# Kmatsuo57/cell-image-analysis

Measured on AMD Instinct MI355X. Metric: cells/sec screened (CAE fwd + recon-MSE + SVM score), 64x64, higher is better.
Workload: dtype f32 (results in the fp32 error class; the contractions run as split 16-bit products on the matrix pipe, fp32 accumulate: conv1..conv6 as 2 fp16 terms x 3 products with exact power-of-two scales from each cell's own data, the PCA GEMM as 3 bf16 terms x 6 products, conv7's 32 -> 16 channel contraction; 1 GPU; BASELINE.json configs[2]: screening inference, 1000000 synthetic 64x64 crops on one GPU, resident in HBM, CAE fwd + recon MSE/MAE + RobustScaler + PCA(100) + 2x OCSVM score on device; cells_per_gpu=1000000, global_cells=1000000, chunk_cells=65536, detector_train_cells=5000, weights=random init (Glorot, non-trivial BN), seed 42, parallelism=dp1

## Files before the change

cell-image-analysis_amd/csrc/conv45_h2.hip:

```cpp
#include "common.hpp"

#include <cstring>

namespace cs {

namespace {

constexpr int G = 8;
constexpr int CH = 32;
constexpr int WP = G + 2;
constexpr int PXB = 64;
constexpr int ROWB = WP * PXB + 32;
constexpr int PLANE = WP * ROWB;
constexpr int WG_PER_CU = 2;

constexpr int C5_OUT = 64;

typedef _Float16 f16x8 __attribute__((ext_vector_type(8)));
typedef _Float16 f16x4 __attribute__((ext_vector_type(4)));
constexpr int H2_OFF_MAX = 2 * PLANE;
constexpr int H2_LDS_BYTES = 2 * PLANE + 16;

__device__ __forceinline__ unsigned int h2_rowmax(unsigned int m)
{
    unsigned int o;
    o = (unsigned int)__builtin_amdgcn_update_dpp(0, (int)m, 0xB1, 0xF, 0xF, true);  m = m > o ? m : o;
    o = (unsigned int)__builtin_amdgcn_update_dpp(0, (int)m, 0x4E, 0xF, 0xF, true);  m = m > o ? m : o;
    o = (unsigned int)__builtin_amdgcn_update_dpp(0, (int)m, 0x124, 0xF, 0xF, true); m = m > o ? m : o;
    o = (unsigned int)__builtin_amdgcn_update_dpp(0, (int)m, 0x128, 0xF, 0xF, true); m = m > o ? m : o;
    return m;
}
__device__ __forceinline__ void h2_scale(unsigned int mbits, float& S, float& invS)
{
    int E = (int)((mbits >> 23) & 0xffu);
    E = E < 40 ? 40 : (E > 254 ? 254 : E);
    S = __builtin_bit_cast(float, (unsigned int)(268 - E) << 23);
    invS = __builtin_bit_cast(float, (unsigned int)(E - 14) << 23);
}
__device__ __forceinline__ void h2_absmax4(const f32x4& v, unsigned int& mx)
{
    const float a = v[0], b = v[1], c = v[2], d = v[3];
    const float m = fmaxf(fmaxf(fabsf(a), fabsf(b)), fmaxf(fabsf(c), fabsf(d)));
    const unsigned int u = __builtin_bit_cast(unsigned int, m);
    mx = mx > u ? mx : u;
}
__device__ __forceinline__ void h2_split_store(char* dst, const f32x4& x, float S)
{
    const f32x4 v = x * S;
    const f16x4 hi = __builtin_convertvector(v, f16x4);
    const f32x4 r = v - __builtin_convertvector(hi, f32x4);
    *(f16x4*)dst = hi;
    *(f16x4*)(dst + PLANE) = __builtin_convertvector(r, f16x4);
}

__global__ __launch_bounds__(256, WG_PER_CU) void conv4_h2_kernel(const float* __restrict__ in, const f16x8* __restrict__ wfrag,
                                                                 const float* __restrict__ ep, float* __restrict__ out,
                                                                 long n_cells, float inv_sw)
{
    extern __shared__ __attribute__((aligned(16))) char smem[];
    unsigned int* const mxw = (unsigned int*)(smem + H2_OFF_MAX);
    const int tid = threadIdx.x;
    const int lane = tid & 63;
    const int wave = __builtin_amdgcn_readfirstlane(tid >> 6);
    const int slice = wave & 1;
    const int th = wave >> 1;
    const int li = lane & 15, kq = lane >> 4;

    f16x8 B[9][2];
#pragma unroll
    for (int t = 0; t < 9; ++t)
#pragma unroll
        for (int p = 0; p < 2; ++p) B[t][p] = wfrag[((slice * 9 + t) * 2 + p) * 64 + lane];
    const int co = slice * 16 + li;
    const float bias = ep[co], bns = ep[CH + co], bnt = ep[2 * CH + co];

    for (int i = tid; i < H2_LDS_BYTES / 16; i += 256) *(f32x4*)(smem + i * 16) = f32x4{0.0f, 0.0f, 0.0f, 0.0f};

    long cell = blockIdx.x;
    if (cell >= n_cells) return;
    f32x4 stg[2];
#pragma unroll
    for (int k = 0; k < 2; ++k) stg[k] = *(const f32x4*)(in + (size_t)cell * (G * G * CH) + (tid + 256 * k) * 4);
    __syncthreads();
    {
        unsigned int mx = 0;
        h2_absmax4(stg[0], mx);
        h2_absmax4(stg[1], mx);
        mx = h2_rowmax(mx);
        if (li == 0) atomicMax(&mxw[0], mx);
    }
    __syncthreads();
    float S, invS;
    h2_scale(mxw[0], S, invS);

    int woff[2];
#pragma unroll
    for (int k = 0; k < 2; ++k) {
        const int idx = tid + 256 * k, px = idx >> 3, c4 = idx & 7;
        woff[k] = ((px >> 3) + 1) * ROWB + ((px & 7) + 1) * PXB + c4 * 8;
    }
    const int abase = (4 * th + (li >> 3)) * ROWB + (li & 7) * PXB + kq * 16;

    for (int it = 0; cell < n_cells; cell += gridDim.x, ++it) {
        const float unscale = invS * inv_sw;
#pragma unroll
        for (int k = 0; k < 2; ++k) h2_split_store(smem + woff[k], stg[k], S);
        __syncthreads();
        if (tid == 0) mxw[it & 1] = 0;
        const long ncell = cell + gridDim.x;
        if (ncell < n_cells) {
#pragma unroll
            for (int k = 0; k < 2; ++k) stg[k] = *(const f32x4*)(in + (size_t)ncell * (G * G * CH) + (tid + 256 * k) * 4);
        }

        f32x4 hi[2] = {{0.0f, 0.0f, 0.0f, 0.0f}, {0.0f, 0.0f, 0.0f, 0.0f}};
        f32x4 lo[2] = {{0.0f, 0.0f, 0.0f, 0.0f}, {0.0f, 0.0f, 0.0f, 0.0f}};
#pragma unroll
        for (int tap = 0; tap < 9; ++tap) {
            const int toff = (tap / 3) * ROWB + (tap % 3) * PXB;
#pragma unroll
            for (int t = 0; t < 2; ++t) {
                const char* a = smem + abase + toff + t * (2 * ROWB);
                const f16x8 a1 = *(const f16x8*)a;
                const f16x8 a2 = *(const f16x8*)(a + PLANE);
                lo[t] = __builtin_amdgcn_mfma_f32_16x16x32_f16(a1, B[tap][1], lo[t], 0, 0, 0);
                hi[t] = __builtin_amdgcn_mfma_f32_16x16x32_f16(a1, B[tap][0], hi[t], 0, 0, 0);
                lo[t] = __builtin_amdgcn_mfma_f32_16x16x32_f16(a2, B[tap][0], lo[t], 0, 0, 0);
            }
        }
#pragma unroll
        for (int t = 0; t < 2; ++t) {
            float* o = out + ((size_t)cell * (G * G) + 16 * (2 * th + t) + 4 * kq) * CH + co;
#pragma unroll
            for (int r = 0; r < 4; ++r) {
                const float v = fmaxf(fmaf(hi[t][r] + lo[t][r], unscale, bias), 0.0f);
                o[r * CH] = fmaf(v, bns, bnt);
            }
        }
        if (ncell < n_cells) {
            unsigned int mx = 0;
            h2_absmax4(stg[0], mx);
            h2_absmax4(stg[1], mx);
            mx = h2_rowmax(mx);
            if (li == 0) atomicMax(&mxw[(it + 1) & 1], mx);
        }
        __syncthreads();
        h2_scale(mxw[(it + 1) & 1], S, invS);
    }
}

__global__ __launch_bounds__(512, 2) void conv5_h2_kernel(const float* __restrict__ in, const f16x8* __restrict__ wfrag,
                                                          const float* __restrict__ ep, float* __restrict__ out, long n_cells, float inv_sw)
{
    extern __shared__ __attribute__((aligned(16))) char smem[];
    unsigned int* const mxw = (unsigned int*)(smem + H2_OFF_MAX);
    const int tid = threadIdx.x;
    const int lane = tid & 63;
    const int wave = __builtin_amdgcn_readfirstlane(tid >> 6);
    const int ph = wave >> 1, pa = ph >> 1, pb = ph & 1;
    const int sp = wave & 1;
    const int li = lane & 15, kq = lane >> 4;

    f16x8 B[4][2][2];
#pragma unroll
    for (int t = 0; t < 4; ++t)
#pragma unroll
        for (int k = 0; k < 2; ++k)
#pragma unroll
            for (int p = 0; p < 2; ++p) B[t][k][p] = wfrag[(((wave * 4 + t) * 2 + k) * 2 + p) * 64 + lane];
    float bias[2], bns[2], bnt[2];
#pragma unroll
    for (int k = 0; k < 2; ++k) {
        const int co = (2 * sp + k) * 16 + li;
        bias[k] = ep[co]; bns[k] = ep[C5_OUT + co]; bnt[k] = ep[2 * C5_OUT + co];
    }

    for (int i = tid; i < H2_LDS_BYTES / 16; i += 512) *(f32x4*)(smem + i * 16) = f32x4{0.0f, 0.0f, 0.0f, 0.0f};

    long cell = blockIdx.x;
    if (cell >= n_cells) return;
    f32x4 stg = *(const f32x4*)(in + (size_t)cell * (G * G * CH) + tid * 4);
    __syncthreads();
    {
        unsigned int mx = 0;
        h2_absmax4(stg, mx);
        mx = h2_rowmax(mx);
        if (li == 0) atomicMax(&mxw[0], mx);
    }
    __syncthreads();
    float S, invS;
    h2_scale(mxw[0], S, invS);
    const int woff = ((tid >> 6) + 1) * ROWB + (((tid >> 3) & 7) + 1) * PXB + (tid & 7) * 8;
    const int abase = ((li >> 3) + pa) * ROWB + ((li & 7) + pb) * PXB + kq * 16;

    for (int it = 0; cell < n_cells; cell += gridDim.x, ++it) {
        const float unscale = invS * inv_sw;
        h2_split_store(smem + woff, stg, S);
        __syncthreads();
        if (tid == 0) mxw[it & 1] = 0;
        const long ncell = cell + gridDim.x;
        if (ncell < n_cells) stg = *(const f32x4*)(in + (size_t)ncell * (G * G * CH) + tid * 4);

        float* obase = out + (((size_t)cell * (2 * G) + pa) * (2 * G) + pb) * C5_OUT + (2 * sp) * 16 + li;
#pragma unroll
        for (int t = 0; t < 4; ++t) {
            f32x4 ah[2] = {{0.0f, 0.0f, 0.0f, 0.0f}, {0.0f, 0.0f, 0.0f, 0.0f}};
            f32x4 al[2] = {{0.0f, 0.0f, 0.0f, 0.0f}, {0.0f, 0.0f, 0.0f, 0.0f}};
#pragma unroll
            for (int tap = 0; tap < 4; ++tap) {
                const char* a = smem + abase + t * (2 * ROWB) + (tap >> 1) * ROWB + (tap & 1) * PXB;
                const f16x8 a1 = *(const f16x8*)a;
                const f16x8 a2 = *(const f16x8*)(a + PLANE);
#pragma unroll
                for (int k = 0; k < 2; ++k) {
                    al[k] = __builtin_amdgcn_mfma_f32_16x16x32_f16(a1, B[tap][k][1], al[k], 0, 0, 0);
                    ah[k] = __builtin_amdgcn_mfma_f32_16x16x32_f16(a1, B[tap][k][0], ah[k], 0, 0, 0);
                    al[k] = __builtin_amdgcn_mfma_f32_16x16x32_f16(a2, B[tap][k][0], al[k], 0, 0, 0);
                }
            }
#pragma unroll
            for (int r = 0; r < 4; ++r) {
                const int i = 4 * kq + r, ys = 2 * t + (i >> 3), xs = i & 7;
                float* o = obase + ((size_t)(2 * ys) * (2 * G) + 2 * xs) * C5_OUT;
#pragma unroll
                for (int k = 0; k < 2; ++k) {
                    const float v = fmaxf(fmaf(ah[k][r] + al[k][r], unscale, bias[k]), 0.0f);
                    o[16 * k] = fmaf(v, bns[k], bnt[k]);
                }
            }
        }
        if (ncell < n_cells) {
            unsigned int mx = 0;
            h2_absmax4(stg, mx);
            mx = h2_rowmax(mx);
            if (li == 0) atomicMax(&mxw[(it + 1) & 1], mx);
        }
        __syncthreads();
        h2_scale(mxw[(it + 1) & 1], S, invS);
    }
}

constexpr int F45_OFF_A = 2 * PLANE;
constexpr int F45_OFF_W4 = 4 * PLANE;
constexpr int F45_W4_BYTES = 2 * 9 * 2 * 64 * 16;
constexpr int F45_OFF_MAX = F45_OFF_W4 + F45_W4_BYTES;
constexpr int F45_LDS_BYTES = F45_OFF_MAX + 16;
static_assert(2 * F45_LDS_BYTES <= 160 * 1024, "two workgroups per CU");

__global__ __launch_bounds__(512, 2) void conv45_h2_kernel(const float* __restrict__ in , const f16x8* __restrict__ w4frag,
                                                           const float* __restrict__ ep4, float inv_sw4, const f16x8* __restrict__ w5frag,
                                                           const float* __restrict__ ep5, float inv_sw5, float* __restrict__ out ,
                                                           long n_cells)
{
    extern __shared__ __attribute__((aligned(16))) char smem[];
    unsigned int* const mxw = (unsigned int*)(smem + F45_OFF_MAX);
    const int tid = threadIdx.x;
    const int lane = tid & 63;
    const int wave = __builtin_amdgcn_readfirstlane(tid >> 6);
    const int li = lane & 15, kq = lane >> 4;
    const int ph = wave >> 1, pa = ph >> 1, pb = ph & 1;
    const int sp = wave & 1;
    const int slice4 = wave & 1, tile4 = wave >> 1;

    f16x8 B[4][2][2];
#pragma unroll
    for (int t = 0; t < 4; ++t)
#pragma unroll
        for (int k = 0; k < 2; ++k)
#pragma unroll
            for (int p = 0; p < 2; ++p) B[t][k][p] = w5frag[(((wave * 4 + t) * 2 + k) * 2 + p) * 64 + lane];
    float bias[2], bns[2], bnt[2];
#pragma unroll
    for (int k = 0; k < 2; ++k) {
        const int co = (2 * sp + k) * 16 + li;
        bias[k] = ep5[co]; bns[k] = ep5[C5_OUT + co]; bnt[k] = ep5[2 * C5_OUT + co];
    }
    const int co4 = slice4 * 16 + li;
    const float bias4 = ep4[co4], bns4 = ep4[CH + co4], bnt4 = ep4[2 * CH + co4];

    for (int i = tid; i < F45_LDS_BYTES / 16; i += 512) *(f32x4*)(smem + i * 16) = f32x4{0.0f, 0.0f, 0.0f, 0.0f};
    __syncthreads();
    for (int i = tid; i < F45_W4_BYTES / 16; i += 512) *(f16x8*)(smem + F45_OFF_W4 + i * 16) = w4frag[i];

    long cell = blockIdx.x;
    if (cell >= n_cells) return;
    f32x4 stg = *(const f32x4*)(in + (size_t)cell * (G * G * CH) + tid * 4);
    {
        unsigned int mx = 0;
        h2_absmax4(stg, mx);
        mx = h2_rowmax(mx);
        if (li == 0) atomicMax(&mxw[0], mx);
    }
    __syncthreads();
    float S3, invS3;
    h2_scale(mxw[0], S3, invS3);
    const int woff = ((tid >> 6) + 1) * ROWB + (((tid >> 3) & 7) + 1) * PXB + (tid & 7) * 8;
    const int abase4 = (2 * tile4 + (li >> 3)) * ROWB + (li & 7) * PXB + kq * 16;
    const char* const w4l = smem + F45_OFF_W4 + (size_t)slice4 * 9 * 2 * 64 * 16 + lane * 16;
    const int abase5 = F45_OFF_A + ((li >> 3) + pa) * ROWB + ((li & 7) + pb) * PXB + kq * 16;

    for (int it = 0; cell < n_cells; cell += gridDim.x, ++it) {
        h2_split_store(smem + woff, stg, S3);
        __syncthreads();
        if (tid == 0) mxw[it & 1] = 0;
        const long ncell = cell + gridDim.x;
        if (ncell < n_cells) stg = *(const f32x4*)(in + (size_t)ncell * (G * G * CH) + tid * 4);

        f32x4 a4v;
        {
            f32x4 hi = {0.0f, 0.0f, 0.0f, 0.0f}, lo = {0.0f, 0.0f, 0.0f, 0.0f};
#pragma unroll
            for (int tap = 0; tap < 9; ++tap) {
                const char* a = smem + abase4 + (tap / 3) * ROWB + (tap % 3) * PXB;
                const f16x8 a1 = *(const f16x8*)a;
                const f16x8 a2 = *(const f16x8*)(a + PLANE);
                const f16x8 bh = *(const f16x8*)(w4l + (tap * 2 + 0) * 1024), bl = *(const f16x8*)(w4l + (tap * 2 + 1) * 1024);
                lo = __builtin_amdgcn_mfma_f32_16x16x32_f16(a1, bl, lo, 0, 0, 0);
                hi = __builtin_amdgcn_mfma_f32_16x16x32_f16(a1, bh, hi, 0, 0, 0);
                lo = __builtin_amdgcn_mfma_f32_16x16x32_f16(a2, bh, lo, 0, 0, 0);
            }
            const float us4 = invS3 * inv_sw4;
            float am = 0.0f;
#pragma unroll
            for (int r = 0; r < 4; ++r) {
                const float v = fmaxf(fmaf(hi[r] + lo[r], us4, bias4), 0.0f);
                a4v[r] = fmaf(v, bns4, bnt4);
                am = fmaxf(am, fabsf(a4v[r]));
            }
            const unsigned int m = h2_rowmax(__builtin_bit_cast(unsigned int, am));
            if (li == 0) atomicMax(&mxw[2 + (it & 1)], m);
        }
        __syncthreads();
        float S4, invS4;
        h2_scale(mxw[2 + (it & 1)], S4, invS4);
        {
#pragma unroll
            for (int r = 0; r < 4; ++r) {
                const int p = 16 * tile4 + 4 * kq + r;
                char* d = smem + F45_OFF_A + ((p >> 3) + 1) * ROWB + ((p & 7) + 1) * PXB + co4 * 2;
                const float v = a4v[r] * S4;
                const _Float16 h = (_Float16)v;
                *(_Float16*)d = h;
                *(_Float16*)(d + PLANE) = (_Float16)(v - (float)h);
            }
        }
        __syncthreads();
        if (tid == 0) mxw[2 + (it & 1)] = 0;

        const float unscale = invS4 * inv_sw5;
        float* obase = out + (((size_t)cell * (2 * G) + pa) * (2 * G) + pb) * C5_OUT + (2 * sp) * 16 + li;
#pragma unroll
        for (int t = 0; t < 4; ++t) {
            f32x4 ah[2] = {{0.0f, 0.0f, 0.0f, 0.0f}, {0.0f, 0.0f, 0.0f, 0.0f}};
            f32x4 al[2] = {{0.0f, 0.0f, 0.0f, 0.0f}, {0.0f, 0.0f, 0.0f, 0.0f}};
#pragma unroll
            for (int tap = 0; tap < 4; ++tap) {
                const char* a = smem + abase5 + t * (2 * ROWB) + (tap >> 1) * ROWB + (tap & 1) * PXB;
                const f16x8 a1 = *(const f16x8*)a;
                const f16x8 a2 = *(const f16x8*)(a + PLANE);
#pragma unroll
                for (int k = 0; k < 2; ++k) {
                    al[k] = __builtin_amdgcn_mfma_f32_16x16x32_f16(a1, B[tap][k][1], al[k], 0, 0, 0);
                    ah[k] = __builtin_amdgcn_mfma_f32_16x16x32_f16(a1, B[tap][k][0], ah[k], 0, 0, 0);
                    al[k] = __builtin_amdgcn_mfma_f32_16x16x32_f16(a2, B[tap][k][0], al[k], 0, 0, 0);
                }
            }
#pragma unroll
            for (int r = 0; r < 4; ++r) {
                const int i = 4 * kq + r, ys = 2 * t + (i >> 3), xs = i & 7;
                float* o = obase + ((size_t)(2 * ys) * (2 * G) + 2 * xs) * C5_OUT;
#pragma unroll
                for (int k = 0; k < 2; ++k) {
                    const float v = fmaxf(fmaf(ah[k][r] + al[k][r], unscale, bias[k]), 0.0f);
                    o[16 * k] = fmaf(v, bns[k], bnt[k]);
                }
            }
        }
        if (ncell < n_cells) {
            unsigned int mx = 0;
            h2_absmax4(stg, mx);
            mx = h2_rowmax(mx);
            if (li == 0) atomicMax(&mxw[(it + 1) & 1], mx);
        }
        __syncthreads();
        h2_scale(mxw[(it + 1) & 1], S3, invS3);
    }
}

}

size_t pack_conv4_f16x2(const float* hwio, uint16_t* dst, float* inv_sw)
{
    const size_t n = (size_t)2 * 9 * 2 * 64 * 8;
    if (!dst) return n;
    const float S = f16x2_weight_scale(hwio, (size_t)9 * CH * CH);
    if (inv_sw) *inv_sw = 1.0f / S;
    for (int s = 0; s < 2; ++s)
        for (int t = 0; t < 9; ++t)
            for (int l = 0; l < 64; ++l)
                for (int j = 0; j < 8; ++j) {
                    const int li = l & 15, kq = l >> 4;
                    uint16_t pl[2];
                    f16x2_split(hwio[((size_t)t * CH + 8 * kq + j) * CH + 16 * s + li], S, pl[0], pl[1]);
                    for (int p = 0; p < 2; ++p) dst[((((size_t)s * 9 + t) * 2 + p) * 64 + l) * 8 + j] = pl[p];
                }
    return n;
}

template <class K>
static hipError_t resident_grid(K kernel, int threads, int lds, int& resident)
{
    int dev = 0, cus = 0, per_cu = 0;
    hipError_t e;
    if ((e = hipGetDevice(&dev)) != hipSuccess) return e;
    if ((e = hipDeviceGetAttribute(&cus, hipDeviceAttributeMultiprocessorCount, dev)) != hipSuccess) return e;
    if ((e = hipOccupancyMaxActiveBlocksPerMultiprocessor(&per_cu, (const void*)kernel, threads, lds)) != hipSuccess) return e;
    resident = cus * (per_cu < 1 ? 1 : per_cu);
    return hipSuccess;
}

hipError_t launch_conv4_h2(const float* in, const uint16_t* wfrag, float inv_sw, const float* ep, float* out, int64_t n_cells, hipStream_t stream)
{
    if (n_cells <= 0) return hipSuccess;
    static int resident = 0;
    if (!resident) {
        hipError_t e = resident_grid(conv4_h2_kernel, 256, H2_LDS_BYTES, resident);
        if (e != hipSuccess) return e;
    }
    const long grid = n_cells < resident ? n_cells : resident;
    hipLaunchKernelGGL(conv4_h2_kernel, dim3((unsigned)grid), dim3(256), H2_LDS_BYTES, stream, in, (const f16x8*)wfrag, ep, out,
                       (long)n_cells, inv_sw);
    return hipGetLastError();
}

size_t pack_conv5_f16x2(const float* weff, uint16_t* dst, float* inv_sw)
{
    const size_t n = (size_t)8 * 4 * 2 * 2 * 64 * 8;
    if (!dst) return n;
    const float S = f16x2_weight_scale(weff, (size_t)16 * CH * C5_OUT);
    if (inv_sw) *inv_sw = 1.0f / S;
    for (int w = 0; w < 8; ++w)
        for (int t = 0; t < 4; ++t)
            for (int k = 0; k < 2; ++k)
                for (int l = 0; l < 64; ++l)
                    for (int j = 0; j < 8; ++j) {
                        const int ph = w >> 1, sp = w & 1, li = l & 15, kq = l >> 4;
                        uint16_t pl[2];
                        f16x2_split(weff[((size_t)(ph * 4 + t) * CH + 8 * kq + j) * C5_OUT + (2 * sp + k) * 16 + li], S, pl[0], pl[1]);
                        for (int p = 0; p < 2; ++p) dst[((((((size_t)w * 4 + t) * 2 + k) * 2 + p) * 64) + l) * 8 + j] = pl[p];
                    }
    return n;
}

hipError_t launch_conv5_h2(const float* in, const uint16_t* wfrag, float inv_sw, const float* ep, float* out, int64_t n_cells, hipStream_t stream)
{
    if (n_cells <= 0) return hipSuccess;
    static int resident = 0;
    if (!resident) {
        hipError_t e = resident_grid(conv5_h2_kernel, 512, H2_LDS_BYTES, resident);
// ... 27 lines not shown
```

cell-image-analysis_amd/csrc/conv_wino_up.hip:

```cpp
#include "common.hpp"

#include <type_traits>

#include <cmath>
#include <cstdlib>
#include <cstring>

namespace cs {

namespace {

template <int HS_, int WS_, int CIN_, int COUT_>
struct WUCfg {
    static constexpr int HS = HS_, WS = WS_, CIN = CIN_, COUT = COUT_;
    static constexpr int HO = 2 * HS, WO = 2 * WS;
    static constexpr int TW = WS / 2;
    static constexpr int SR = 2 * (16 / TW);
    static constexpr int R = SR + 2, WP = WS + 2;
    static constexpr int PS = CIN + 4;
    static constexpr int STRIP = R * WP * PS * 4;
    static constexpr int LDS = 2 * STRIP;
    static constexpr int NGRP = HS / SR;
    static constexpr int NQ = CIN / 16, KS = CIN / 4;
    static constexpr int NSW = COUT / 32;
// ... 329 lines not shown
                    t1 = __builtin_amdgcn_mfma_f32_16x16x4f32(a10[s], wc[s], t1, 0, 0, 0);
                }
#pragma unroll
                for (int s = 0; s < 4; ++s) {
                    t0 = __builtin_amdgcn_mfma_f32_16x16x4f32(a01[s], wc[4 + s], t0, 0, 0, 0);
                    t1 = __builtin_amdgcn_mfma_f32_16x16x4f32(a11[s], wc[4 + s], t1, 0, 0, 0);
                }
                float* tw = tb + ((((8 * grp + wave) & (F67::TSLOTS - 1)) * F67::TWD) + 4 * kq + 1) * 16 + li;
#pragma unroll
                for (int r = 0; r < 4; ++r) { tw[r * 16] = t0[r]; tw[(16 + r) * 16] = t1[r]; }
            }
            if (has_next) {
#pragma unroll
                for (int j = 0; j < C::NLD; ++j) wu_store<C>(nstrip, ngrp * C::SR, j, rsub, loff, stg[j]);
            }
            __syncthreads();
            if constexpr (DIAG) { const unsigned long long t = wu_stamp(); dg[3] += t - dt; dt = t; }
            const int px = lane & 1, xh = (lane >> 1) + px;
#pragma unroll
            for (int h = 0; h < 2; ++h) {
                const int k = wave + 8 * h;
                const int y = 8 * grp + (k >> 1), e = k & 1;
                if (2 * y - 1 + e < 0) continue;
                const int nb = ((1 - e) * 2 + px) * 4;
                const float* ra = tb + (((y - 1) & (F67::TSLOTS - 1)) * F67::TWD + xh) * 16 + nb;
                const float* rb = tb + ((y & (F67::TSLOTS - 1)) * F67::TWD + xh) * 16 + nb;
                float ta0 = ra[0], ta1 = ra[16 + 1];
                const float tb0 = rb[2], tb1 = rb[16 + 3];
                if (y == 0) { ta0 = 0.0f; ta1 = 0.0f; }
                const float v = ((ta0 + ta1) + (tb0 + tb1)) + b7;
                const float rr = f67_sigmoid(v);
                const float d = xv[h] - rr;
                s2 = fmaf(d, d, s2);
                s1 += fabsf(d);
            }
            if (grp == C::NGRP - 1 && wave == 0) {
                const int nb = (2 + px) * 4;
                const float* ra = tb + ((31 & (F67::TSLOTS - 1)) * F67::TWD + xh) * 16 + nb;
                const float v = (ra[0] + ra[16 + 1]) + b7;
                const float rr = f67_sigmoid(v);
                const float d = xtail - rr;
                s2 = fmaf(d, d, s2);
                s1 += fabsf(d);
            }
            if constexpr (DIAG) {
                asm volatile("" ::"v"(s2), "v"(s1));
                const unsigned long long t = wu_stamp(); dg[4] += t - dt; dt = t;
            }
            buf ^= 1;
        }
#pragma unroll
        for (int off = 32; off > 0; off >>= 1) {
            s2 += __shfl_down(s2, off, 64);
            s1 += __shfl_down(s1, off, 64);
        }
        if (lane == 0) {
            errpart[((size_t)cell * F67::NPARTS + wave) * 2 + 0] = s2;
            errpart[((size_t)cell * F67::NPARTS + wave) * 2 + 1] = s1;
        }
    }
    if constexpr (DIAG) {
        if (lane == 0) {
#pragma unroll
            for (int k = 0; k < 5; ++k) diag[((size_t)blockIdx.x * 8 + wave) * 5 + k] = dg[k];
        }
    }
}

struct F67T {
    static constexpr int TW = 36;
    static constexpr int T_BYTES = F67::TSLOTS * 16 * TW * 4;
};

typedef _Float16 f16x8 __attribute__((ext_vector_type(8)));
typedef _Float16 f16x4 __attribute__((ext_vector_type(4)));

struct F67H {
    static constexpr int PLB = 2 * 64;
    static constexpr int PXB = 2 * PLB + 32;
    static constexpr int ROWB = 18 * PXB;
    static constexpr int STRIP = 6 * ROWB;
    static constexpr int TW = F67T::TW;
    static constexpr int T_BYTES = F67T::T_BYTES;
    static constexpr int PA = 40;
    static constexpr int A6_BYTES = 8 * 32 * PA * 4;
    static constexpr int WP = 40;
    static constexpr int W_BYTES = 16 * WP * 4;
    static constexpr int OFF_MAX = STRIP + A6_BYTES + T_BYTES + W_BYTES;
    static constexpr int LDS = OFF_MAX + 16;
    static_assert(LDS <= 160 * 1024 && STRIP % 16 == 0, "LDS budget");
};

__device__ __forceinline__ unsigned int h2_rowmax(unsigned int m)
{
    unsigned int o;
    o = (unsigned int)__builtin_amdgcn_update_dpp(0, (int)m, 0xB1, 0xF, 0xF, true);  m = m > o ? m : o;
    o = (unsigned int)__builtin_amdgcn_update_dpp(0, (int)m, 0x4E, 0xF, 0xF, true);  m = m > o ? m : o;
    o = (unsigned int)__builtin_amdgcn_update_dpp(0, (int)m, 0x124, 0xF, 0xF, true); m = m > o ? m : o;
    o = (unsigned int)__builtin_amdgcn_update_dpp(0, (int)m, 0x128, 0xF, 0xF, true); m = m > o ? m : o;
    return m;
}

__device__ __forceinline__ void h2_scale(unsigned int mbits, float& S, float& invS)
{
    int E = (int)((mbits >> 23) & 0xffu);
    E = E < 40 ? 40 : (E > 254 ? 254 : E);
    S = __builtin_bit_cast(float, (unsigned int)(268 - E) << 23);
    invS = __builtin_bit_cast(float, (unsigned int)(E - 14) << 23);
}

__device__ __forceinline__ void h2_split4(const f32x4& x, float S, f16x4& hi, f16x4& lo)
{
    const f32x4 v = x * S;
    hi = __builtin_convertvector(v, f16x4);
    const f32x4 r = v - __builtin_convertvector(hi, f32x4);
    lo = __builtin_convertvector(r, f16x4);
}

__device__ __forceinline__ void h2_store(char* strip, int j, int rsub, int loffb, const f32x4& v, float S)
{
    const int r = rsub + WUL6::RPP * j;
    f16x4 hi, lo;
    h2_split4(v, S, hi, lo);
    char* d = strip + r * F67H::ROWB + loffb;
    *(f16x4*)d = hi;
    *(f16x4*)(d + F67H::PLB) = lo;
}

__device__ __forceinline__ f32x4 h2_prep(int y0, int j, int rsub, f32x4 v, unsigned int& mx)
{
    const int sy = y0 - 1 + rsub + WUL6::RPP * j;
    if (sy < 0 || sy >= WUL6::HS) v = f32x4{0.0f, 0.0f, 0.0f, 0.0f};
    const float a = v[0], b = v[1], c = v[2], d = v[3];
    const unsigned int u = __builtin_bit_cast(unsigned int, fmaxf(fmaxf(fabsf(a), fabsf(b)), fmaxf(fabsf(c), fabsf(d))));
    mx = mx > u ? mx : u;
    return v;
}

template <bool DIAG>
__global__ __launch_bounds__(WUL6::THREADS, 2) void conv67_h2_kernel(
    const float* __restrict__ in , const f16x8* __restrict__ wfrag, const float* __restrict__ ep ,
    const float* __restrict__ x , const float* __restrict__ weff ,
    const float* __restrict__ b7p, float* __restrict__ errpart , long n_cells, float inv_sw,
    unsigned long long* __restrict__ diag)
{
    using C = WUL6;
    static_assert(C::NLD == 3 && C::RPP == 2 && C::R == 6 && C::EPR == 256, "row-wise staging constants");
    unsigned long long dg[5] = {0, 0, 0, 0, 0}, dt = 0;
    extern __shared__ __attribute__((aligned(16))) char smem[];
    float* a6s = (float*)(smem + F67H::STRIP);
    float* tb = (float*)(smem + F67H::STRIP + F67H::A6_BYTES);
    float* wl = (float*)(smem + F67H::STRIP + F67H::A6_BYTES + F67H::T_BYTES);
    unsigned int* mxw = (unsigned int*)(smem + F67H::OFF_MAX);
    const int tid = threadIdx.x, lane = tid & 63;
    const int wave = __builtin_amdgcn_readfirstlane(tid >> 6);
    const int ph = wave >> 1, wsl = wave & 1;
    const int pa = ph >> 1, pb = ph & 1;
    const int li = lane & 15, kq = lane >> 4;

    f16x8 B[4][2][2];
#pragma unroll
    for (int t = 0; t < 4; ++t)
#pragma unroll
        for (int k = 0; k < 2; ++k)
#pragma unroll
            for (int p = 0; p < 2; ++p) B[t][k][p] = wfrag[(((wave * 4 + t) * 2 + k) * 2 + p) * 64 + lane];
    const int co = wsl * 16 + li;
    const int cosw = co ^ ((kq & 1) << 4);
    const float bias = ep[co], bns = ep[C::COUT + co], bnt = ep[2 * C::COUT + co];
    const float b7 = b7p[0];

    const long first = blockIdx.x;
    if (first >= n_cells) return;
    const int se = tid & (C::EPR - 1), rsub = tid / C::EPR;
    const int spx = se / C::C4, sc4 = se & (C::C4 - 1);
    const int goff = spx * C::CIN + sc4 * 4;
    const int loffb = (spx + 1) * F67H::PXB + sc4 * 8;
    auto cell_ptr = [&](long cell) { return in + (size_t)cell * C::HS * C::WS * C::CIN; };
    for (int i = tid; i < F67H::LDS / 16; i += C::THREADS) ((f32x4*)smem)[i] = f32x4{0.0f, 0.0f, 0.0f, 0.0f};
    __syncthreads();
    wl[(tid >> 5) * F67H::WP + (tid & 31)] = weff[tid];
    float unscale;
    {
        f32x4 stg[C::NLD];
        unsigned int mx = 0;
#pragma unroll
        for (int j = 0; j < C::NLD; ++j) stg[j] = h2_prep(0, j, rsub, wu_load<C>(cell_ptr(first), 0, j, rsub, goff), mx);
        mx = h2_rowmax(mx);
        if (li == 0) atomicMax(&mxw[0], mx);
        __syncthreads();
        float S, invS;
        h2_scale(mxw[0], S, invS);
        unscale = invS * inv_sw;
#pragma unroll
        for (int j = 0; j < C::NLD; ++j) h2_store(smem, j, rsub, loffb, stg[j], S);
    }
    __syncthreads();
    if (tid == 0) mxw[0] = 0;
    const char* abase = smem + (pa * 18 + li + pb) * F67H::PXB + kq * 16;

    int strip_no = 0;
    for (long cell = first; cell < n_cells; cell += gridDim.x) {
        const float* xc = x + (size_t)cell * 64 * 64;
        float s2 = 0.0f, s1 = 0.0f;
#pragma unroll 1
        for (int grp = 0; grp < C::NGRP; ++grp) {
            const long ncell = grp < C::NGRP - 1 ? cell : cell + gridDim.x;
            const int ngrp = grp < C::NGRP - 1 ? grp + 1 : 0;
            const bool has_next = ncell < n_cells;
            ++strip_no;
            unsigned int* const mword = mxw + (strip_no & 1);

            if constexpr (DIAG) dt = wu_stamp();
            f32x4 stg[C::NLD];
            if (has_next) {
#pragma unroll
                for (int j = 0; j < C::NLD; ++j) stg[j] = wu_load<C>(cell_ptr(ncell), ngrp * C::SR, j, rsub, goff);
            }
            float xv[2];
#pragma unroll
            for (int h = 0; h < 2; ++h) {
                const int k = wave + 8 * h, o = 2 * (8 * grp + (k >> 1)) - 1 + (k & 1);
                xv[h] = xc[(o < 0 ? 0 : o) * 64 + lane];
            }
            float xtail = 0.0f;
            if (grp == C::NGRP - 1 && wave == 0) xtail = xc[63 * 64 + lane];

            if constexpr (DIAG) { const unsigned long long t = wu_stamp(); dg[0] += t - dt; dt = t; }
            f32x4 ah[4], al[4];
#pragma unroll
            for (int t = 0; t < 4; ++t) ah[t] = al[t] = f32x4{0.0f, 0.0f, 0.0f, 0.0f};
            auto rd = [&](int f, f16x8 (&a)[2]) {
                const int sr = f >> 2, rx = (f >> 1) & 1, k = f & 1;
                const char* p = abase + sr * F67H::ROWB + rx * F67H::PXB + k * 64;
                a[0] = *(const f16x8*)p;
                a[1] = *(const f16x8*)(p + F67H::PLB);
            };
            auto mac3 = [&](const f16x8 (&a)[2], const f16x8 (&b)[2], f32x4& dh, f32x4& dl) {
                dl = __builtin_amdgcn_mfma_f32_16x16x32_f16(a[0], b[1], dl, 0, 0, 0);
                dh = __builtin_amdgcn_mfma_f32_16x16x32_f16(a[0], b[0], dh, 0, 0, 0);
                dl = __builtin_amdgcn_mfma_f32_16x16x32_f16(a[1], b[0], dl, 0, 0, 0);
            };
            {
                f16x8 a[2];
                rd(0, a);
                __builtin_amdgcn_sched_group_barrier(0x100, 2, 0);
#pragma unroll
                for (int f = 0; f < 20; ++f) {
                    const int sr = f >> 2, rx = (f >> 1) & 1, k = f & 1;
                    f16x8 an[2] = {a[0], a[1]};
                    if (f + 1 < 20) rd(f + 1, an);
                    if (sr < 4) mac3(a, B[rx][k], ah[sr], al[sr]);
                    if (sr > 0) mac3(a, B[2 + rx][k], ah[sr - 1], al[sr - 1]);
                    a[0] = an[0]; a[1] = an[1];
                    __builtin_amdgcn_sched_group_barrier(0x100, 2, 0);
                    if (sr > 0 && sr < 4) __builtin_amdgcn_sched_group_barrier(0x008, 6, 0);
                    else __builtin_amdgcn_sched_group_barrier(0x008, 3, 0);
                }
            }
            if constexpr (DIAG) {
                asm volatile("" ::"v"(ah[0][0]), "v"(al[3][3]));
                const unsigned long long t = wu_stamp(); dg[1] += t - dt; dt = t;
            }
#pragma unroll
            for (int t = 0; t < 4; ++t)
#pragma unroll
                for (int r = 0; r < 4; ++r) {
                    const float v = fmaxf(fmaf(ah[t][r] + al[t][r], unscale, bias), 0.0f);
                    a6s[((2 * t + pa) * 32 + 2 * (4 * kq + r) + pb) * F67H::PA + cosw] = fmaf(v, bns, bnt);
                }
            if (has_next) {
                unsigned int mx = 0;
#pragma unroll
                for (int j = 0; j < C::NLD; ++j) stg[j] = h2_prep(ngrp * C::SR, j, rsub, stg[j], mx);
                mx = h2_rowmax(mx);
                if (li == 0) atomicMax(mword, mx);
            }
            __syncthreads();
            if constexpr (DIAG) { const unsigned long long t = wu_stamp(); dg[2] += t - dt; dt = t; }
            {
                const int wrow = 4 * ((li >> 3) | (((li >> 2) & 1) << 1)) + (li & 3);
                float wc[8];
                *(f32x4*)&wc[0] = *(const f32x4*)(wl + wrow * F67H::WP + 4 * kq);
                *(f32x4*)&wc[4] = *(const f32x4*)(wl + wrow * F67H::WP + 4 * kq + 16);
                const int pix = 4 * (li & 3) + (li >> 2), sw = ((li >> 1) & 1) << 4;
                const float* ap = a6s + (wave * 32 + pix) * F67H::PA + 4 * kq;
                const f32x4 a00 = *(const f32x4*)(ap + sw), a01 = *(const f32x4*)(ap + (sw ^ 16));
                const f32x4 a10 = *(const f32x4*)(ap + 16 * F67H::PA + sw), a11 = *(const f32x4*)(ap + 16 * F67H::PA + (sw ^ 16));
                f32x4 t0 = f32x4{0.0f, 0.0f, 0.0f, 0.0f}, t1 = t0;
#pragma unroll
                for (int s = 0; s < 4; ++s) {
                    t0 = __builtin_amdgcn_mfma_f32_16x16x4f32(wc[s], a00[s], t0, 0, 0, 0);
                    t1 = __builtin_amdgcn_mfma_f32_16x16x4f32(wc[s], a10[s], t1, 0, 0, 0);
                }
#pragma unroll
                for (int s = 0; s < 4; ++s) {
                    t0 = __builtin_amdgcn_mfma_f32_16x16x4f32(wc[4 + s], a01[s], t0, 0, 0, 0);
                    t1 = __builtin_amdgcn_mfma_f32_16x16x4f32(wc[4 + s], a11[s], t1, 0, 0, 0);
                }
                const int rblk = kq == 0 ? 0 : (kq == 1 ? 3 : (kq == 2 ? 1 : 2));
                float* tw = tb + ((((8 * grp + wave) & (F67::TSLOTS - 1)) * 16) + 4 * rblk) * F67H::TW + pix + 1 - (kq >> 1);
#pragma unroll
                for (int r = 0; r < 4; ++r) { tw[r * F67H::TW] = t0[r]; tw[r * F67H::TW + 16] = t1[r]; }
            }
            if (has_next) {
                float S, invS;
                h2_scale(*mword, S, invS);
                unscale = invS * inv_sw;
#pragma unroll
                for (int j = 0; j < C::NLD; ++j) h2_store(smem, j, rsub, loffb, stg[j], S);
            }
            __syncthreads();
            if (tid == 0) *mword = 0;
            if constexpr (DIAG) { const unsigned long long t = wu_stamp(); dg[3] += t - dt; dt = t; }
            const int px = lane & 1, xh = lane >> 1;
#pragma unroll
            for (int h = 0; h < 2; ++h) {
                const int k = wave + 8 * h;
                const int y = 8 * grp + (k >> 1), e = k & 1;
                if (2 * y - 1 + e < 0) continue;
                const int nb = (e ? px : 3 - px) * 4;
                const float* ra = tb + ((((y - 1) & (F67::TSLOTS - 1)) * 16) + nb) * F67H::TW + xh;
                const float* rb = tb + (((y & (F67::TSLOTS - 1)) * 16) + nb) * F67H::TW + xh;
                float ta0 = ra[0], ta1 = ra[F67H::TW + 1];
                const float tb0 = rb[2 * F67H::TW], tb1 = rb[3 * F67H::TW + 1];
                if (y == 0) { ta0 = 0.0f; ta1 = 0.0f; }
                const float v = ((ta0 + ta1) + (tb0 + tb1)) + b7;
                const float rr = f67_sigmoid(v);
                const float d = xv[h] - rr;
                s2 = fmaf(d, d, s2);
                s1 += fabsf(d);
            }
            if (grp == C::NGRP - 1 && wave == 0) {
                const int nb = (3 - px) * 4;
                const float* ra = tb + (((31 & (F67::TSLOTS - 1)) * 16) + nb) * F67H::TW + xh;
                const float v = (ra[0] + ra[F67H::TW + 1]) + b7;
                const float rr = f67_sigmoid(v);
                const float d = xtail - rr;
                s2 = fmaf(d, d, s2);
                s1 += fabsf(d);
            }
            if constexpr (DIAG) {
                asm volatile("" ::"v"(s2), "v"(s1));
                const unsigned long long t = wu_stamp(); dg[4] += t - dt; dt = t;
            }
        }
#pragma unroll
        for (int off = 32; off > 0; off >>= 1) {
            s2 += __shfl_down(s2, off, 64);
            s1 += __shfl_down(s1, off, 64);
        }
        if (lane == 0) {
            errpart[((size_t)cell * F67::NPARTS + wave) * 2 + 0] = s2;
            errpart[((size_t)cell * F67::NPARTS + wave) * 2 + 1] = s1;
        }
    }
    if constexpr (DIAG) {
        if (lane == 0) {
#pragma unroll
            for (int k = 0; k < 5; ++k) diag[((size_t)blockIdx.x * 8 + wave) * 5 + k] = dg[k];
        }
    }
}

template <class C>
size_t pack_frags(const float* hwio, float* dst)
{
    const size_t total = (size_t)8 * C::NB * 64;
    if (!dst) return total;
// ... 194 lines not shown
```

Measured before the change: 5.612 million cells/s.

## Swap MFMA operands so conv epilogues write channel-contiguous float4 stores

Every f16 MFMA in conv4, conv5, fused conv4+5 and conv6 now takes the weight fragment as the A operand and activations as B. Each lane then holds four consecutive output channels for a single pixel, instead of four pixels for one channel. This lets the BN/ReLU epilogue issue one 16-byte vector store per accumulator rather than four scattered scalar stores, both to global memory and to the conv6->conv7 LDS staging. The staging buffer's padding grows from 40 to 48 with an XOR swizzle so the conv7 reads stay bank-friendly. It also changes LDS footprint and per-lane bias/BN register usage (now four values each).

```diff
diff --git a/cell-image-analysis_amd/csrc/conv45_h2.hip b/cell-image-analysis_amd/csrc/conv45_h2.hip
--- a/cell-image-analysis_amd/csrc/conv45_h2.hip
+++ b/cell-image-analysis_amd/csrc/conv45_h2.hip
@@ -51,6 +51,18 @@
     const f32x4 r = v - __builtin_convertvector(hi, f32x4);
     *(f16x4*)dst = hi;
     *(f16x4*)(dst + PLANE) = __builtin_convertvector(r, f16x4);
+}
+
+__device__ __forceinline__ f32x4 h2_epilogue4(const f32x4& hi, const f32x4& lo, float unscale, const f32x4& bias, const f32x4& bns,
+                                              const f32x4& bnt)
+{
+    f32x4 y;
+#pragma unroll
+    for (int r = 0; r < 4; ++r) {
+        const float v = fmaxf(fmaf(hi[r] + lo[r], unscale, bias[r]), 0.0f);
+        y[r] = fmaf(v, bns[r], bnt[r]);
+    }
+    return y;
 }
 
 __global__ __launch_bounds__(256, WG_PER_CU) void conv4_h2_kernel(const float* __restrict__ in, const f16x8* __restrict__ wfrag,
@@ -71,8 +83,10 @@
     for (int t = 0; t < 9; ++t)
 #pragma unroll
         for (int p = 0; p < 2; ++p) B[t][p] = wfrag[((slice * 9 + t) * 2 + p) * 64 + lane];
-    const int co = slice * 16 + li;
-    const float bias = ep[co], bns = ep[CH + co], bnt = ep[2 * CH + co];
+    const int co = slice * 16 + 4 * kq;
+    f32x4 bias, bns, bnt;
+#pragma unroll
+    for (int r = 0; r < 4; ++r) { bias[r] = ep[co + r]; bns[r] = ep[CH + co + r]; bnt[r] = ep[2 * CH + co + r]; }
 
     for (int i = tid; i < H2_LDS_BYTES / 16; i += 256) *(f32x4*)(smem + i * 16) = f32x4{0.0f, 0.0f, 0.0f, 0.0f};
 
@@ -123,20 +137,14 @@
                 const char* a = smem + abase + toff + t * (2 * ROWB);
                 const f16x8 a1 = *(const f16x8*)a;
                 const f16x8 a2 = *(const f16x8*)(a + PLANE);
-                lo[t] = __builtin_amdgcn_mfma_f32_16x16x32_f16(a1, B[tap][1], lo[t], 0, 0, 0);
-                hi[t] = __builtin_amdgcn_mfma_f32_16x16x32_f16(a1, B[tap][0], hi[t], 0, 0, 0);
-                lo[t] = __builtin_amdgcn_mfma_f32_16x16x32_f16(a2, B[tap][0], lo[t], 0, 0, 0);
+                lo[t] = __builtin_amdgcn_mfma_f32_16x16x32_f16(B[tap][1], a1, lo[t], 0, 0, 0);
+                hi[t] = __builtin_amdgcn_mfma_f32_16x16x32_f16(B[tap][0], a1, hi[t], 0, 0, 0);
+                lo[t] = __builtin_amdgcn_mfma_f32_16x16x32_f16(B[tap][0], a2, lo[t], 0, 0, 0);
             }
         }
 #pragma unroll
-        for (int t = 0; t < 2; ++t) {
-            float* o = out + ((size_t)cell * (G * G) + 16 * (2 * th + t) + 4 * kq) * CH + co;
-#pragma unroll
-            for (int r = 0; r < 4; ++r) {
-                const float v = fmaxf(fmaf(hi[t][r] + lo[t][r], unscale, bias), 0.0f);
-                o[r * CH] = fmaf(v, bns, bnt);
-            }
-        }
+        for (int t = 0; t < 2; ++t)
+            *(f32x4*)(out + ((size_t)cell * (G * G) + 16 * (2 * th + t) + li) * CH + co) = h2_epilogue4(hi[t], lo[t], unscale, bias, bns, bnt);
         if (ncell < n_cells) {
             unsigned int mx = 0;
             h2_absmax4(stg[0], mx);
@@ -168,12 +176,14 @@
         for (int k = 0; k < 2; ++k)
 #pragma unroll
             for (int p = 0; p < 2; ++p) B[t][k][p] = wfrag[(((wave * 4 + t) * 2 + k) * 2 + p) * 64 + lane];
-    float bias[2], bns[2], bnt[2];
-#pragma unroll
-    for (int k = 0; k < 2; ++k) {
-        const int co = (2 * sp + k) * 16 + li;
-        bias[k] = ep[co]; bns[k] = ep[C5_OUT + co]; bnt[k] = ep[2 * C5_OUT + co];
-    }
+    f32x4 bias[2], bns[2], bnt[2];
+#pragma unroll
+    for (int k = 0; k < 2; ++k)
+#pragma unroll
+        for (int r = 0; r < 4; ++r) {
+            const int co = (2 * sp + k) * 16 + 4 * kq + r;
+            bias[k][r] = ep[co]; bns[k][r] = ep[C5_OUT + co]; bnt[k][r] = ep[2 * C5_OUT + co];
+        }
 
     for (int i = tid; i < H2_LDS_BYTES / 16; i += 512) *(f32x4*)(smem + i * 16) = f32x4{0.0f, 0.0f, 0.0f, 0.0f};
 
@@ -192,6 +202,7 @@
     h2_scale(mxw[0], S, invS);
     const int woff = ((tid >> 6) + 1) * ROWB + (((tid >> 3) & 7) + 1) * PXB + (tid & 7) * 8;
     const int abase = ((li >> 3) + pa) * ROWB + ((li & 7) + pb) * PXB + kq * 16;
+    const int opix = (2 * (li >> 3) * (2 * G) + 2 * (li & 7)) * C5_OUT + (2 * sp) * 16 + 4 * kq;
 
     for (int it = 0; cell < n_cells; cell += gridDim.x, ++it) {
         const float unscale = invS * inv_sw;
@@ -201,7 +212,7 @@
         const long ncell = cell + gridDim.x;
         if (ncell < n_cells) stg = *(const f32x4*)(in + (size_t)ncell * (G * G * CH) + tid * 4);
 
-        float* obase = out + (((size_t)cell * (2 * G) + pa) * (2 * G) + pb) * C5_OUT + (2 * sp) * 16 + li;
+        float* obase = out + (((size_t)cell * (2 * G) + pa) * (2 * G) + pb) * C5_OUT + opix;
 #pragma unroll
         for (int t = 0; t < 4; ++t) {
             f32x4 ah[2] = {{0.0f, 0.0f, 0.0f, 0.0f}, {0.0f, 0.0f, 0.0f, 0.0f}};
@@ -213,21 +224,14 @@
                 const f16x8 a2 = *(const f16x8*)(a + PLANE);
 #pragma unroll
                 for (int k = 0; k < 2; ++k) {
-                    al[k] = __builtin_amdgcn_mfma_f32_16x16x32_f16(a1, B[tap][k][1], al[k], 0, 0, 0);
-                    ah[k] = __builtin_amdgcn_mfma_f32_16x16x32_f16(a1, B[tap][k][0], ah[k], 0, 0, 0);
-                    al[k] = __builtin_amdgcn_mfma_f32_16x16x32_f16(a2, B[tap][k][0], al[k], 0, 0, 0);
+                    al[k] = __builtin_amdgcn_mfma_f32_16x16x32_f16(B[tap][k][1], a1, al[k], 0, 0, 0);
+                    ah[k] = __builtin_amdgcn_mfma_f32_16x16x32_f16(B[tap][k][0], a1, ah[k], 0, 0, 0);
+                    al[k] = __builtin_amdgcn_mfma_f32_16x16x32_f16(B[tap][k][0], a2, al[k], 0, 0, 0);
                 }
             }
-#pragma unroll
-            for (int r = 0; r < 4; ++r) {
-                const int i = 4 * kq + r, ys = 2 * t + (i >> 3), xs = i & 7;
-                float* o = obase + ((size_t)(2 * ys) * (2 * G) + 2 * xs) * C5_OUT;
-#pragma unroll
-                for (int k = 0; k < 2; ++k) {
-                    const float v = fmaxf(fmaf(ah[k][r] + al[k][r], unscale, bias[k]), 0.0f);
-                    o[16 * k] = fmaf(v, bns[k], bnt[k]);
-                }
-            }
+            float* o = obase + (size_t)(4 * t) * (2 * G) * C5_OUT;
+#pragma unroll
+            for (int k = 0; k < 2; ++k) *(f32x4*)(o + 16 * k) = h2_epilogue4(ah[k], al[k], unscale, bias[k], bns[k], bnt[k]);
         }
         if (ncell < n_cells) {
             unsigned int mx = 0;
@@ -269,14 +273,18 @@
         for (int k = 0; k < 2; ++k)
 #pragma unroll
             for (int p = 0; p < 2; ++p) B[t][k][p] = w5frag[(((wave * 4 + t) * 2 + k) * 2 + p) * 64 + lane];
-    float bias[2], bns[2], bnt[2];
-#pragma unroll
-    for (int k = 0; k < 2; ++k) {
-        const int co = (2 * sp + k) * 16 + li;
-        bias[k] = ep5[co]; bns[k] = ep5[C5_OUT + co]; bnt[k] = ep5[2 * C5_OUT + co];
-    }
-    const int co4 = slice4 * 16 + li;
-    const float bias4 = ep4[co4], bns4 = ep4[CH + co4], bnt4 = ep4[2 * CH + co4];
+    f32x4 bias[2], bns[2], bnt[2];
+#pragma unroll
+    for (int k = 0; k < 2; ++k)
+#pragma unroll
+        for (int r = 0; r < 4; ++r) {
+            const int co = (2 * sp + k) * 16 + 4 * kq + r;
+            bias[k][r] = ep5[co]; bns[k][r] = ep5[C5_OUT + co]; bnt[k][r] = ep5[2 * C5_OUT + co];
+        }
+    const int co4 = slice4 * 16 + 4 * kq;
+    f32x4 bias4, bns4, bnt4;
+#pragma unroll
+    for (int r = 0; r < 4; ++r) { bias4[r] = ep4[co4 + r]; bns4[r] = ep4[CH + co4 + r]; bnt4[r] = ep4[2 * CH + co4 + r]; }
 
     for (int i = tid; i < F45_LDS_BYTES / 16; i += 512) *(f32x4*)(smem + i * 16) = f32x4{0.0f, 0.0f, 0.0f, 0.0f};
     __syncthreads();
@@ -298,6 +306,8 @@
     const int abase4 = (2 * tile4 + (li >> 3)) * ROWB + (li & 7) * PXB + kq * 16;
     const char* const w4l = smem + F45_OFF_W4 + (size_t)slice4 * 9 * 2 * 64 * 16 + lane * 16;
     const int abase5 = F45_OFF_A + ((li >> 3) + pa) * ROWB + ((li & 7) + pb) * PXB + kq * 16;
+    const int opix = (2 * (li >> 3) * (2 * G) + 2 * (li & 7)) * C5_OUT + (2 * sp) * 16 + 4 * kq;
+    const int a4off = F45_OFF_A + (2 * tile4 + (li >> 3) + 1) * ROWB + ((li & 7) + 1) * PXB + co4 * 2;
 
     for (int it = 0; cell < n_cells; cell += gridDim.x, ++it) {
         h2_split_store(smem + woff, stg, S3);
@@ -315,40 +325,25 @@
                 const f16x8 a1 = *(const f16x8*)a;
                 const f16x8 a2 = *(const f16x8*)(a + PLANE);
                 const f16x8 bh = *(const f16x8*)(w4l + (tap * 2 + 0) * 1024), bl = *(const f16x8*)(w4l + (tap * 2 + 1) * 1024);
-                lo = __builtin_amdgcn_mfma_f32_16x16x32_f16(a1, bl, lo, 0, 0, 0);
-                hi = __builtin_amdgcn_mfma_f32_16x16x32_f16(a1, bh, hi, 0, 0, 0);
-                lo = __builtin_amdgcn_mfma_f32_16x16x32_f16(a2, bh, lo, 0, 0, 0);
+                lo = __builtin_amdgcn_mfma_f32_16x16x32_f16(bl, a1, lo, 0, 0, 0);
+                hi = __builtin_amdgcn_mfma_f32_16x16x32_f16(bh, a1, hi, 0, 0, 0);
+                lo = __builtin_amdgcn_mfma_f32_16x16x32_f16(bh, a2, lo, 0, 0, 0);
             }
-            const float us4 = invS3 * inv_sw4;
-            float am = 0.0f;
-#pragma unroll
-            for (int r = 0; r < 4; ++r) {
-                const float v = fmaxf(fmaf(hi[r] + lo[r], us4, bias4), 0.0f);
-                a4v[r] = fmaf(v, bns4, bnt4);
-                am = fmaxf(am, fabsf(a4v[r]));
-            }
-            const unsigned int m = h2_rowmax(__builtin_bit_cast(unsigned int, am));
+            a4v = h2_epilogue4(hi, lo, invS3 * inv_sw4, bias4, bns4, bnt4);
+            unsigned int am = 0;
+            h2_absmax4(a4v, am);
+            const unsigned int m = h2_rowmax(am);
             if (li == 0) atomicMax(&mxw[2 + (it & 1)], m);
         }
         __syncthreads();
         float S4, invS4;
         h2_scale(mxw[2 + (it & 1)], S4, invS4);
-        {
-#pragma unroll
-            for (int r = 0; r < 4; ++r) {
-                const int p = 16 * tile4 + 4 * kq + r;
-                char* d = smem + F45_OFF_A + ((p >> 3) + 1) * ROWB + ((p & 7) + 1) * PXB + co4 * 2;
-                const float v = a4v[r] * S4;
-                const _Float16 h = (_Float16)v;
-                *(_Float16*)d = h;
-                *(_Float16*)(d + PLANE) = (_Float16)(v - (float)h);
-            }
-        }
+        h2_split_store(smem + a4off, a4v, S4);
         __syncthreads();
         if (tid == 0) mxw[2 + (it & 1)] = 0;
 
         const float unscale = invS4 * inv_sw5;
-        float* obase = out + (((size_t)cell * (2 * G) + pa) * (2 * G) + pb) * C5_OUT + (2 * sp) * 16 + li;
+        float* obase = out + (((size_t)cell * (2 * G) + pa) * (2 * G) + pb) * C5_OUT + opix;
 #pragma unroll
         for (int t = 0; t < 4; ++t) {
             f32x4 ah[2] = {{0.0f, 0.0f, 0.0f, 0.0f}, {0.0f, 0.0f, 0.0f, 0.0f}};
@@ -360,21 +355,14 @@
                 const f16x8 a2 = *(const f16x8*)(a + PLANE);
 #pragma unroll
                 for (int k = 0; k < 2; ++k) {
-                    al[k] = __builtin_amdgcn_mfma_f32_16x16x32_f16(a1, B[tap][k][1], al[k], 0, 0, 0);
-                    ah[k] = __builtin_amdgcn_mfma_f32_16x16x32_f16(a1, B[tap][k][0], ah[k], 0, 0, 0);
-                    al[k] = __builtin_amdgcn_mfma_f32_16x16x32_f16(a2, B[tap][k][0], al[k], 0, 0, 0);
+                    al[k] = __builtin_amdgcn_mfma_f32_16x16x32_f16(B[tap][k][1], a1, al[k], 0, 0, 0);
+                    ah[k] = __builtin_amdgcn_mfma_f32_16x16x32_f16(B[tap][k][0], a1, ah[k], 0, 0, 0);
+                    al[k] = __builtin_amdgcn_mfma_f32_16x16x32_f16(B[tap][k][0], a2, al[k], 0, 0, 0);
                 }
             }
-#pragma unroll
-            for (int r = 0; r < 4; ++r) {
-                const int i = 4 * kq + r, ys = 2 * t + (i >> 3), xs = i & 7;
-                float* o = obase + ((size_t)(2 * ys) * (2 * G) + 2 * xs) * C5_OUT;
-#pragma unroll
-                for (int k = 0; k < 2; ++k) {
-                    const float v = fmaxf(fmaf(ah[k][r] + al[k][r], unscale, bias[k]), 0.0f);
-                    o[16 * k] = fmaf(v, bns[k], bnt[k]);
-                }
-            }
+            float* o = obase + (size_t)(4 * t) * (2 * G) * C5_OUT;
+#pragma unroll
+            for (int k = 0; k < 2; ++k) *(f32x4*)(o + 16 * k) = h2_epilogue4(ah[k], al[k], unscale, bias[k], bns[k], bnt[k]);
         }
         if (ncell < n_cells) {
             unsigned int mx = 0;
diff --git a/cell-image-analysis_amd/csrc/conv_wino_up.hip b/cell-image-analysis_amd/csrc/conv_wino_up.hip
--- a/cell-image-analysis_amd/csrc/conv_wino_up.hip
+++ b/cell-image-analysis_amd/csrc/conv_wino_up.hip
@@ -435,7 +435,7 @@
     static constexpr int STRIP = 6 * ROWB;
     static constexpr int TW = F67T::TW;
     static constexpr int T_BYTES = F67T::T_BYTES;
-    static constexpr int PA = 40;
+    static constexpr int PA = 48;
     static constexpr int A6_BYTES = 8 * 32 * PA * 4;
     static constexpr int WP = 40;
     static constexpr int W_BYTES = 16 * WP * 4;
@@ -518,9 +518,11 @@
         for (int k = 0; k < 2; ++k)
 #pragma unroll
             for (int p = 0; p < 2; ++p) B[t][k][p] = wfrag[(((wave * 4 + t) * 2 + k) * 2 + p) * 64 + lane];
-    const int co = wsl * 16 + li;
-    const int cosw = co ^ ((kq & 1) << 4);
-    const float bias = ep[co], bns = ep[C::COUT + co], bnt = ep[2 * C::COUT + co];
+    const int co = wsl * 16 + 4 * kq;
+    const int a6off = (pa * 32 + 2 * li + pb) * F67H::PA + 4 * (((co >> 2) ^ li) & 7);
+    f32x4 bias, bns, bnt;
+#pragma unroll
+    for (int r = 0; r < 4; ++r) { bias[r] = ep[co + r]; bns[r] = ep[C::COUT + co + r]; bnt[r] = ep[2 * C::COUT + co + r]; }
     const float b7 = b7p[0];
 
     const long first = blockIdx.x;
@@ -590,9 +592,9 @@
                 a[1] = *(const f16x8*)(p + F67H::PLB);
             };
             auto mac3 = [&](const f16x8 (&a)[2], const f16x8 (&b)[2], f32x4& dh, f32x4& dl) {
-                dl = __builtin_amdgcn_mfma_f32_16x16x32_f16(a[0], b[1], dl, 0, 0, 0);
-                dh = __builtin_amdgcn_mfma_f32_16x16x32_f16(a[0], b[0], dh, 0, 0, 0);
-                dl = __builtin_amdgcn_mfma_f32_16x16x32_f16(a[1], b[0], dl, 0, 0, 0);
+                dl = __builtin_amdgcn_mfma_f32_16x16x32_f16(b[1], a[0], dl, 0, 0, 0);
+                dh = __builtin_amdgcn_mfma_f32_16x16x32_f16(b[0], a[0], dh, 0, 0, 0);
+                dl = __builtin_amdgcn_mfma_f32_16x16x32_f16(b[0], a[1], dl, 0, 0, 0);
             };
             {
                 f16x8 a[2];
@@ -616,12 +618,15 @@
                 const unsigned long long t = wu_stamp(); dg[1] += t - dt; dt = t;
             }
 #pragma unroll
-            for (int t = 0; t < 4; ++t)
+            for (int t = 0; t < 4; ++t) {
+                f32x4 y;
 #pragma unroll
                 for (int r = 0; r < 4; ++r) {
-                    const float v = fmaxf(fmaf(ah[t][r] + al[t][r], unscale, bias), 0.0f);
-                    a6s[((2 * t + pa) * 32 + 2 * (4 * kq + r) + pb) * F67H::PA + cosw] = fmaf(v, bns, bnt);
+                    const float v = fmaxf(fmaf(ah[t][r] + al[t][r], unscale, bias[r]), 0.0f);
+                    y[r] = fmaf(v, bns[r], bnt[r]);
                 }
+                *(f32x4*)(a6s + a6off + 2 * t * 32 * F67H::PA) = y;
+            }
             if (has_next) {
                 unsigned int mx = 0;
 #pragma unroll
@@ -636,8 +641,8 @@
                 float wc[8];
                 *(f32x4*)&wc[0] = *(const f32x4*)(wl + wrow * F67H::WP + 4 * kq);
                 *(f32x4*)&wc[4] = *(const f32x4*)(wl + wrow * F67H::WP + 4 * kq + 16);
-                const int pix = 4 * (li & 3) + (li >> 2), sw = ((li >> 1) & 1) << 4;
-                const float* ap = a6s + (wave * 32 + pix) * F67H::PA + 4 * kq;
+                const int pix = 4 * (li & 3) + (li >> 2), sw = 4 * (kq ^ ((pix >> 1) & 7));
+                const float* ap = a6s + (wave * 32 + pix) * F67H::PA;
                 const f32x4 a00 = *(const f32x4*)(ap + sw), a01 = *(const f32x4*)(ap + (sw ^ 16));
                 const f32x4 a10 = *(const f32x4*)(ap + 16 * F67H::PA + sw), a11 = *(const f32x4*)(ap + 16 * F67H::PA + (sw ^ 16));
                 f32x4 t0 = f32x4{0.0f, 0.0f, 0.0f, 0.0f}, t1 = t0;
```

After: 5.392 million cells/s. -3.9%, worse.
